# Nicholasli1995/EgoNet

Hardware: AMD Instinct MI355X
Metric: crops/sec (256x256, heatmap+decode+lift) (higher is better)
Workload: dtype f32; 1 GPU; configs[1]: batch=64 256x256 crops/GPU, HRNet-W48 heatmap head forward + soft decode + affine + FC lifter + pose solve; global_batch=64, weights=synthetic (egonet_amd.synth, seeded per key), parallelism=replicas x1, crops sharded by rank, no collective, ranks=1, backend=none, launch_lanes=1

## Files before the change

egonet_amd/csrc/conv_s2r.hip:

```cpp
#include <stdlib.h>

#include "conv_common.h"

typedef __attribute__((address_space(3))) void* lds_ptr_s2r_t;

namespace {
constexpr int S2_NW = 3, S2_NTH = 64 * S2_NW;
constexpr int S2_CIN = 48, S2_CG = 48;
constexpr int S2_TP = 16, S2_TH = 2, S2_TW = 8;
constexpr int S2_NSLAB = 27;
constexpr int S2_LDS = S2_NSLAB * 1024;
}

__device__ __forceinline__ void s2r_dma16(u32x4 r, unsigned lds_addr, unsigned voff) {
  asm volatile("s_mov_b32 m0, %0\n\ts_nop 0\n\tbuffer_load_dwordx4 %1, %2, 0 offen lds"
               :
               : "s"(lds_addr), "v"(voff), "s"(r)
               : "m0", "memory");
}

__global__ __launch_bounds__(S2_NTH, 4) void conv_s2r_kernel(ConvArgs a) {
  extern __shared__ float4 s2_smem[];
  const unsigned lds0 = (unsigned)(__UINTPTR_TYPE__)(lds_ptr_s2r_t)s2_smem;
  const char* smc = reinterpret_cast<const char*>(s2_smem);

  const int tid = threadIdx.x, lane = tid & 63;
  const int wave = __builtin_amdgcn_readfirstlane(tid >> 6);
  const int li = lane & 15, kq = lane >> 4;
  const int Co = a.Cout, CoP = a.CoutP;
  const int ncg = Co / S2_CG;
  const int tiles_x = a.Wo / S2_TW, tiles_y = a.Ho / S2_TH;
  const int ntile = a.N * tiles_y * tiles_x;
  const int nitem = ntile * ncg;
  const int gsz = (int)gridDim.x;
  const int cg = (int)blockIdx.x % ncg;
  const int co = cg * S2_CG + 16 * wave + li;

  const unsigned long long xaddr = reinterpret_cast<unsigned long long>(a.x);
  const u32x4 rx = {(unsigned)xaddr, (unsigned)(xaddr >> 32) & 0xffffu, (unsigned)((size_t)a.N * a.H * a.W * S2_CIN * 4),
                    0x00020000u};
  const __amdgpu_buffer_rsrc_t ry =
      __builtin_amdgcn_make_buffer_rsrc(a.y, 0, (unsigned)((size_t)a.N * a.Ho * a.Wo * Co * 4), 0x00020000);

  f32x4 b[9][3];
#pragma unroll
  for (int tap = 0; tap < 9; ++tap)
#pragma unroll
    for (int ch = 0; ch < 3; ++ch)
      b[tap][ch] = *reinterpret_cast<const f32x4*>(a.w + ((size_t)((ch * 9 + tap) * 4 + kq) * CoP + co) * 4);
  const float sc = a.scale[co], sh = a.shift[co];
  const float lo = (a.act & EGN_ACT_MASK) == EGN_ACT_RELU ? 0.f : -__builtin_inff();

  const int drow = lane >> 2;
  const int dquad = (lane & 3) ^ (((drow >> 3) & 1) << 1);
  const unsigned frag = (unsigned)(li * 64 + ((kq ^ (((li >> 3) & 1) << 1)) << 4));

  for (int item = blockIdx.x; item < nitem; item += gsz) {
    const int t = item / ncg;
    const int tx = t % tiles_x, tyn = t / tiles_x;
    const int ty = tyn % tiles_y, n = tyn / tiles_y;
    const int oy = S2_TH * ty + (drow >> 3), ox = S2_TW * tx + (drow & 7);
    const int iy0 = 2 * oy - 1, ix0 = 2 * ox - 1;
    const int pixoff = (((n * a.H + iy0) * a.W + ix0) * S2_CIN + 4 * dquad) * 4;
    __builtin_amdgcn_s_barrier();
    asm volatile("" ::: "memory");
#pragma unroll
    for (int j = 0; j < 9; ++j) {
      const int p = 9 * wave + j;
      const int tap = p / 3, ch = p - 3 * tap;
      const int ky = tap / 3, kx = tap - 3 * ky;
      const bool ok = (unsigned)(iy0 + ky) < (unsigned)a.H && (unsigned)(ix0 + kx) < (unsigned)a.W;
      const unsigned voff = ok ? (unsigned)(pixoff + ((ky * a.W + kx) * S2_CIN + 16 * ch) * 4) : EGN_OOB;
      s2r_dma16(rx, lds0 + (unsigned)p * 1024u, voff);
    }
    asm volatile("s_waitcnt vmcnt(0)" ::: "memory");
    __builtin_amdgcn_s_barrier();
    asm volatile("" ::: "memory");
    f32x4 acc = {0.f, 0.f, 0.f, 0.f};
#pragma unroll
    for (int tap = 0; tap < 9; ++tap)
#pragma unroll
      for (int ch = 0; ch < 3; ++ch) {
        const f32x4 af = *reinterpret_cast<const f32x4*>(smc + (tap * 3 + ch) * 1024 + frag);
#pragma unroll
        for (int s = 0; s < 4; ++s) acc = __builtin_amdgcn_mfma_f32_16x16x4f32(af[s], b[tap][ch][s], acc, 0, 0, 0);
      }
    const unsigned vo = (unsigned)((((n * a.Ho + S2_TH * ty + (kq >> 1)) * a.Wo + S2_TW * tx + 4 * (kq & 1)) * Co + co) * 4);
#pragma unroll
    for (int r = 0; r < 4; ++r) {
      const float v = fmaxf(__builtin_fmaf(acc[r], sc, sh), lo);
      __builtin_amdgcn_raw_buffer_store_b32(__builtin_bit_cast(unsigned, v), ry, vo, (unsigned)(r * Co * 4), 0);
    }
  }
}

bool egn_conv_s2r_applies(const ConvArgs& a) {
  const int act = a.act & EGN_ACT_MASK;
  return a.KH == 3 && a.KW == 3 && a.stride == 2 && a.pad == 1 && a.Cin == S2_CIN && a.cs_in == S2_CIN &&
         a.Cout % S2_CG == 0 && a.cs_out == a.Cout && !a.out_nchw && a.res == nullptr && !(a.act & EGN_ACT_RES_AFTER) &&
         (act == EGN_ACT_NONE || act == EGN_ACT_RELU) && a.H % 2 == 0 && a.W % 2 == 0 && a.Ho % S2_TH == 0 &&
         a.Wo % S2_TW == 0 && a.stats == nullptr;
}
size_t egn_conv_s2r_lds_bytes() { return S2_LDS; }

int egn_conv_launch_s2r(const ConvArgs& a, hipStream_t stream) {
  if (!egn_conv_s2r_applies(a)) return EGN_E_BADARG;
  static bool raised[EGN_MAX_DEVICES];
  static int cus = 0;
  if (egn_first_use_on_device(raised))
    EGN_CHECK_HIP(hipFuncSetAttribute(reinterpret_cast<const void*>(&conv_s2r_kernel), hipFuncAttributeMaxDynamicSharedMemorySize,
                                      S2_LDS));
  if (!cus) {
    int dev = 0;
    hipDeviceProp_t prop;
    if (hipGetDevice(&dev) == hipSuccess && hipGetDeviceProperties(&prop, dev) == hipSuccess) cus = prop.multiProcessorCount;
    if (cus <= 0) cus = 256;
  }
  const int ncg = a.Cout / S2_CG;
  const int nitem = a.N * (a.Ho / S2_TH) * (a.Wo / S2_TW) * ncg;
  static const int bpc = [] { const char* e = getenv("EGN_S2R_BPC"); const int v = e ? atoi(e) : 5; return v >= 1 && v <= 5 ? v : 5; }();
  int grid = bpc * cus / ncg * ncg;
  if (grid <= 0) grid = ncg;
  if (nitem < grid) grid = (nitem + ncg - 1) / ncg * ncg;
  hipLaunchKernelGGL(conv_s2r_kernel, dim3(grid), dim3(S2_NTH), S2_LDS, stream, a);
  return (int)hipGetLastError();
}
```

Before: 5058 crops/s.

## Pipeline stride-2 conv LDS DMA per kernel row across tiles

Restructures the persistent stride-2 conv loop so input DMA is issued one kernel row at a time, and the next tile's rows 0 and 1 are prefetched while the current tile's MFMAs run. Waits use partial vmcnt counts instead of draining all loads before compute. The goal is to hide global-to-LDS load latency behind matrix work. In exchange it relies on precise vmcnt accounting that includes the output stores, and the bounds checks are simplified to top and left edges only.

After: 5075 crops/s, median of 6. No clear change (+0.3%).

```diff
diff --git a/egonet_amd/csrc/conv_s2r.hip b/egonet_amd/csrc/conv_s2r.hip
--- a/egonet_amd/csrc/conv_s2r.hip
+++ b/egonet_amd/csrc/conv_s2r.hip
@@ -55,43 +55,80 @@
   const int dquad = (lane & 3) ^ (((drow >> 3) & 1) << 1);
   const unsigned frag = (unsigned)(li * 64 + ((kq ^ (((li >> 3) & 1) << 1)) << 4));
 
-  for (int item = blockIdx.x; item < nitem; item += gsz) {
-    const int t = item / ncg;
-    const int tx = t % tiles_x, tyn = t / tiles_x;
-    const int ty = tyn % tiles_y, n = tyn / tiles_y;
-    const int oy = S2_TH * ty + (drow >> 3), ox = S2_TW * tx + (drow & 7);
-    const int iy0 = 2 * oy - 1, ix0 = 2 * ox - 1;
-    const int pixoff = (((n * a.H + iy0) * a.W + ix0) * S2_CIN + 4 * dquad) * 4;
-    __builtin_amdgcn_s_barrier();
-    asm volatile("" ::: "memory");
+  int item = blockIdx.x;
+  if (item >= nitem) return;
+
+  const unsigned dlane = (unsigned)(((2 * (drow >> 3) * a.W + 2 * (drow & 7)) * S2_CIN + 4 * dquad) * 4);
+  const bool ltop = (drow >> 3) == 0, lleft = (drow & 7) == 0 && wave == 0;
+  const int rowb = a.W * S2_CIN * 4;
+  int dn, dty, dtx, dbase;
+  auto locate = [&](int it) {
+    const int t = it / ncg;
+    dtx = t % tiles_x;
+    const int tyn = t / tiles_x;
+    dty = tyn % tiles_y;
+    dn = tyn / tiles_y;
+    dbase = ((dn * a.H + 2 * S2_TH * dty - 1) * a.W + 2 * S2_TW * dtx - 1 + wave) * S2_CIN * 4;
+  };
+  auto issue_row = [&](int ky) {
+    const bool out = (lleft && dtx == 0) || (ky == 0 && ltop && dty == 0);
+    const unsigned voff = out ? EGN_OOB : dlane + (unsigned)(dbase + ky * rowb);
 #pragma unroll
-    for (int j = 0; j < 9; ++j) {
-      const int p = 9 * wave + j;
-      const int tap = p / 3, ch = p - 3 * tap;
-      const int ky = tap / 3, kx = tap - 3 * ky;
-      const bool ok = (unsigned)(iy0 + ky) < (unsigned)a.H && (unsigned)(ix0 + kx) < (unsigned)a.W;
-      const unsigned voff = ok ? (unsigned)(pixoff + ((ky * a.W + kx) * S2_CIN + 16 * ch) * 4) : EGN_OOB;
-      s2r_dma16(rx, lds0 + (unsigned)p * 1024u, voff);
-    }
-    asm volatile("s_waitcnt vmcnt(0)" ::: "memory");
-    __builtin_amdgcn_s_barrier();
-    asm volatile("" ::: "memory");
-    f32x4 acc = {0.f, 0.f, 0.f, 0.f};
+    for (int ch = 0; ch < 3; ++ch)
+      s2r_dma16(rx, lds0 + (unsigned)(9 * ky + 3 * wave + ch) * 1024u, voff + 64u * (unsigned)ch);
+  };
+  f32x4 acc;
+  auto mma_row = [&](int ky) {
 #pragma unroll
-    for (int tap = 0; tap < 9; ++tap)
+    for (int kx = 0; kx < 3; ++kx)
 #pragma unroll
       for (int ch = 0; ch < 3; ++ch) {
-        const f32x4 af = *reinterpret_cast<const f32x4*>(smc + (tap * 3 + ch) * 1024 + frag);
+        const f32x4 af = *reinterpret_cast<const f32x4*>(smc + ((ky * 3 + kx) * 3 + ch) * 1024 + frag);
 #pragma unroll
-        for (int s = 0; s < 4; ++s) acc = __builtin_amdgcn_mfma_f32_16x16x4f32(af[s], b[tap][ch][s], acc, 0, 0, 0);
+        for (int s = 0; s < 4; ++s) acc = __builtin_amdgcn_mfma_f32_16x16x4f32(af[s], b[ky * 3 + kx][ch][s], acc, 0, 0, 0);
       }
+  };
+#define S2R_VMCNT(N) asm volatile("s_waitcnt vmcnt(" #N ")" ::: "memory")
+#define S2R_BARRIER()                  \
+  do {                                 \
+    __builtin_amdgcn_s_barrier();      \
+    asm volatile("" ::: "memory");     \
+  } while (0)
+
+  locate(item);
+  issue_row(0);
+  issue_row(1);
+  for (bool first = true;; first = false) {
+    const int n = dn, ty = dty, tx = dtx;
+    const int nxt = item + gsz;
+    const bool more = nxt < nitem;
+    acc = f32x4{0.f, 0.f, 0.f, 0.f};
+    if (first) S2R_VMCNT(3); else S2R_VMCNT(7);
+    S2R_BARRIER();
+    issue_row(2);
+    mma_row(0);
+    if (first) S2R_VMCNT(3); else S2R_VMCNT(7);
+    S2R_BARRIER();
+    if (more) {
+      locate(nxt);
+      issue_row(0);
+    }
+    mma_row(1);
+    if (more) S2R_VMCNT(3); else S2R_VMCNT(0);
+    S2R_BARRIER();
+    if (more) issue_row(1);
+    mma_row(2);
     const unsigned vo = (unsigned)((((n * a.Ho + S2_TH * ty + (kq >> 1)) * a.Wo + S2_TW * tx + 4 * (kq & 1)) * Co + co) * 4);
 #pragma unroll
     for (int r = 0; r < 4; ++r) {
       const float v = fmaxf(__builtin_fmaf(acc[r], sc, sh), lo);
       __builtin_amdgcn_raw_buffer_store_b32(__builtin_bit_cast(unsigned, v), ry, vo, (unsigned)(r * Co * 4), 0);
     }
+    if (!more) break;
+    item = nxt;
   }
+#undef S2R_VMCNT
+#undef S2R_BARRIER
 }
 
 bool egn_conv_s2r_applies(const ConvArgs& a) {
```
